# USTC-StarTeam/DR4SR

Measured on AMD Instinct MI355X. Metric: training sequences/sec, SASRec d=64 L=50, higher is better.
Workload: dtype f32; 1 GPU; SASRec on amazon-toys-shaped synthetic rows (BASELINE configs[1]): N=11925, L=50, d=64, 2 layers, 2 heads, FFN 128, dropout 0.50, B=256 rows/GPU/step, toys histogram (10.9% valid) seqlen; global_batch=256, seq_len=50, parallelism=dp1, hip_graph=True, steps_per_graph=30

## Files before the change

dr4sr_amd/csrc/common.h:

```cpp
#pragma once
#include <hip/hip_runtime.h>
#include <stdint.h>
#include "../../include/dr4sr_hip.h"
#include "../../include/dr4sr_hip_hooks.h"
#include <stdlib.h>
#include <string.h>

#include <atomic>
#include <mutex>
int dr4sr_env_generation();
std::mutex& dr4sr_env_mutex();
#define DR4SR_ENV(NAME) ([]() -> const char* {                                                   \
    static std::atomic<int> gen_{-1}; static bool set_ = false; static char buf_[256];           \
    const int cur_ = dr4sr_env_generation();                                                     \
    if (gen_.load(std::memory_order_acquire) != cur_) {                                          \
        std::lock_guard<std::mutex> lk_(dr4sr_env_mutex());                                      \
        if (gen_.load(std::memory_order_relaxed) != cur_) { const char* e_ = getenv(NAME); set_ = e_ != nullptr; \
            if (e_) { strncpy(buf_, e_, sizeof(buf_) - 1); buf_[sizeof(buf_) - 1] = 0; }         \
            gen_.store(cur_, std::memory_order_release); } }                                     \
    return set_ ? buf_ : nullptr; }())

#ifdef DR4SR_EXPERIMENTS
#define DR4SR_XENV(NAME) DR4SR_ENV(NAME)
#else
// ... 506 lines not shown
        const int lane = threadIdx.x & 63, w = threadIdx.x >> 6, r16 = lane & 15, g = lane >> 4;
#pragma unroll
        for (int i = 0; i < N / 64; ++i) {
            const int col = (w + 4 * i) * 16 + r16;
            const float bv = bias ? bias[col] : 0.f;
#pragma unroll
            for (int r = 0; r < BM / 16; ++r)
#pragma unroll
                for (int q = 0; q < 4; ++q) Cs[(r * 16 + 4 * g + q) * ldc + col] = t.a[r][i][q] + bv;
        }
    }
}
template <int BM, int N>
__device__ __forceinline__ void tile_to_global(const TileAcc<BM, N>& t, float* __restrict__ C, int ldc, const float* __restrict__ bias,
                                               int t0, int T) {
    if constexpr (BM == 64) acc_to_global(t.a, C, ldc, bias, t0, T);
    else {
        const int lane = threadIdx.x & 63, w = threadIdx.x >> 6, r16 = lane & 15, g = lane >> 4;
#pragma unroll
        for (int i = 0; i < N / 64; ++i) {
            const int col = (w + 4 * i) * 16 + r16;
            const float bv = bias ? bias[col] : 0.f;
#pragma unroll
            for (int r = 0; r < BM / 16; ++r)
#pragma unroll
                for (int q = 0; q < 4; ++q) {
                    const int tt = t0 + r * 16 + 4 * g + q;
                    if (tt < T) C[(size_t)tt * ldc + col] = t.a[r][i][q] + bv;
                }
        }
    }
}

template <int BM, int K>
__device__ __forceinline__ void load_tile_bm(float* __restrict__ As, int lda, const float* __restrict__ G, int ldg, int t0, int T) {
    constexpr int C4 = K / 4;
    for (int i = threadIdx.x; i < BM * C4; i += 256) {
        const int row = i / C4, c = (i % C4) * 4;
        float4 v = make_float4(0.f, 0.f, 0.f, 0.f);
        if (t0 + row < T) v = ld4(G + (size_t)(t0 + row) * ldg + c);
        st4(As + row * lda + c, v);
    }
}

template <int K>
__device__ __forceinline__ void load_tile(float* __restrict__ As, int lda, const float* __restrict__ G,
                                          int ldg, int t0, int T) {
    constexpr int C4 = K / 4;
    for (int i = threadIdx.x; i < 64 * C4; i += 256) {
        const int row = i / C4, c = (i % C4) * 4;
        float4 v = make_float4(0.f, 0.f, 0.f, 0.f);
        if (t0 + row < T) v = ld4(G + (size_t)(t0 + row) * ldg + c);
        st4(As + row * lda + c, v);
    }
}

template <int NV, bool DPP = false>
__device__ __forceinline__ void ln_stats16(const float4 (&v)[NV], float& mean, float& rstd, float eps) {
    constexpr float invD = 1.0f / (64 * NV);
    float s = 0.f;
#pragma unroll
    for (int j = 0; j < NV; ++j) s += (v[j].x + v[j].y) + (v[j].z + v[j].w);
    mean = group16_sum_sel<DPP>(s) * invD;
    float q = 0.f;
#pragma unroll
    for (int j = 0; j < NV; ++j) {
// ... 66 lines not shown
```

dr4sr_amd/csrc/linear.hip:

```cpp
#include "common.h"
#include "kernels.h"
#include <cstdlib>
#define STAMP(i) do { if (A.stamps && blockIdx.x == 0 && threadIdx.x == 0) A.stamps[i] = __builtin_amdgcn_s_memtime(); } while (0)

extern __shared__ __attribute__((aligned(16))) float smem[];

__global__ __launch_bounds__(256) void k_transpose(const float* __restrict__ params, float* __restrict__ wT,
                                                   int64_t o_in, int64_t o_out, int64_t o_w1, int64_t o_w2,
                                                   int64_t layer_stride, int64_t wT_stride, int D, int F) {
    const int m = blockIdx.y, layer = blockIdx.z;
    const float* src;
    float* dst = wT + layer * wT_stride;
    int R, C;
    if (m == 0) { src = params + o_in + layer * layer_stride; R = 3 * D; C = D; }
    else if (m == 1) { src = params + o_out + layer * layer_stride; R = D; C = D; dst += 3 * D * D; }
    else if (m == 2) { src = params + o_w1 + layer * layer_stride; R = F; C = D; dst += 4 * D * D; }
    else { src = params + o_w2 + layer * layer_stride; R = D; C = F; dst += 4 * D * D + D * F; }
    for (int i = blockIdx.x * 256 + threadIdx.x; i < R * C; i += gridDim.x * 256) {
        const int r = i / C, c = i % C;
        dst[c * R + r] = src[i];
    }
}

int launch_transpose_weights(const dr4sr_sasrec_plan* p, const Workspace& ws, hipStream_t s) {
// ... 166 lines not shown
        const int layer = j / E4, q = j % E4, e = 4 * q;
        int64_t so; int C, m_off;
        if (e < 3 * D * D) { so = o_in; C = D; m_off = 0; }
        else if (e < 4 * D * D) { so = o_out; C = D; m_off = 3 * D * D; }
        else if (e < 4 * D * D + F * D) { so = o_w1; C = D; m_off = 4 * D * D; }
        else { so = o_w2; C = F; m_off = 4 * D * D + F * D; }
        const int K = C, idx = q - m_off / 4, lane = idx & 63, tq = idx >> 6, ci = tq % (K / 16), ct = tq / (K / 16);
        const int n = ct * 16 + (lane & 15), k0 = (lane >> 4) * (K / 4) + 4 * ci;
        st4(out + (size_t)layer * E + e, ld4(A.E + so + layer * LSTR + (size_t)n * C + k0));
    }
}
template <int D>
__global__ __launch_bounds__(256) void k_wfrag_write(const EmbQkvArgs A) { wfrag_image_write<D>(A); }
int launch_wfrag_write(const dr4sr_sasrec_plan* p, const Workspace& ws, hipStream_t s) {
    EmbQkvArgs A{};
    A.E = p->params + ws.off[0]; A.W = p->params + poff(ws, 0, P_IN_W); A.wf_layers = p->n_layer;
    A.sp = reinterpret_cast<const unsigned short*>(ws.wfrag);
    hipLaunchKernelGGL(k_wfrag_write<128>, dim3(64), dim3(256), 0, s, A);
    return DR4SR_LAUNCH_CHECK();
}

template <int BM, int D>
__global__ __launch_bounds__(256) void k_embqkv_fwd(const EmbQkvArgs A) {
    constexpr int N = 3 * D, LDA = D + 4, LPT = D / 4, TPB = 256 / LPT;
    if constexpr (BM == 16 && D == 128) { if (A.wf_layers > 0) wfrag_image_write<D>(A); }
    const int T = A.state[DR4SR_STATE_T], t0 = xcd_tile(T, BM, A.xcd) * BM;
    if (t0 >= T) return;
    float* As = smem;
    const int c = (threadIdx.x % LPT) * 4;
    const bool dodrop = A.training && A.p > 0.f;
    const RngKey rk = make_rng(A.seed, (uint32_t)A.state[DR4SR_STATE_RNGSTEP], A.p);
    constexpr bool PFE = BM == 16 && D == 64;
    WFragT<PFE ? D : 16, PFE ? N : 64> f_in;
    if constexpr (PFE) wfrag_load(f_in, A.W, D);
    const int bh = A.tile_seq[t0 >> 4];
#pragma unroll
    for (int r0 = 0; r0 < BM; r0 += TPB) {
        const int r = r0 + threadIdx.x / LPT, t = t0 + r;
        if (r < BM) {
            float4 o = make_float4(0.f, 0.f, 0.f, 0.f);
            if (t < T) {
                const int b = find_seq_from(A.cu, A.B, t, bh), pos = t - A.cu[b];
                const int64_t row = A.rows ? A.rows[b] : b;
                int64_t id = A.idx[row * A.L + pos];
                if (A.idx32 && c == 0) A.idx32[t] = (id > 0 && id < A.n_items) ? (int)id : 0;
                if (A.tok && c == 0) A.tok[t] = make_int2(t - pos, b | ((A.cu[b + 1] - A.cu[b]) << 20) | (id == 0 ? 1 << 30 : 0));
                id = id < 0 ? 0 : (id >= A.n_items ? A.n_items - 1 : id);
                o = ld4(A.E + id * D + c);
                const float4 pe = ld4(A.P + (size_t)pos * D + c);
                o = make_float4(o.x + pe.x, o.y + pe.y, o.z + pe.z, o.w + pe.w);
                if (dodrop) {
                    const float4 m = drop4(rk, DR4SR_SITE_EMB, ((uint64_t)b * A.L + pos) * D + c);
                    o.x *= m.x; o.y *= m.y; o.z *= m.z; o.w *= m.w;
                }
                st4(A.X + (size_t)t * D + c, o);
            }
            st4(As + r * LDA + c, o);
        }
    }
    lds_barrier();
    TileAcc<BM, N> acc;
    tile_zero(acc);
    if constexpr (PFE) tile_mma_frag<BM, D, N>(As, LDA, f_in, acc);
    else tile_gemm<D == 128 && BM == 32, BM, D, N>(As, LDA, A.W, D, false, A.sp, WSplitGeo<D, 128>::E, 0, acc);
    tile_to_global<BM, N>(acc, A.QKV, N, A.bias, t0, T);
    if (A.dqkv_zero) zero_kv_rows<BM, D>(A.dqkv_zero, t0, T);
}

int launch_embqkv_fwd(const dr4sr_sasrec_plan* p, const Workspace& ws, int training, hipStream_t s) {
    const int D = p->D, bm = tile_rows(ws);
    const size_t lds = sizeof(float) * bm * (D + 4);
    dim3 grid((ws.Tmax + bm - 1) / bm), blk(256);
    EmbQkvArgs A;
    A.E = p->params + ws.off[0]; A.P = p->params + ws.off[1]; A.idx = p->in_item_id; A.rows = p->rows; A.cu = ws.cu; A.tile_seq = ws.tile_seq; A.X = ws.X[0];
    A.W = p->params + poff(ws, 0, P_IN_W); A.bias = p->params + poff(ws, 0, P_IN_B); A.QKV = ws.layer[0].qkv; A.state = p->state;
    A.B = p->B; A.L = p->L; A.n_items = p->n_items; A.training = training; A.seed = p->seed; A.p = p->p_drop;
    A.idx32 = de_owner_mode(ws) ? ws.idx32 : nullptr;
    A.sp = wsplit_of(p, ws, 0); A.wf_layers = 0;
    if (wfrag_img_on(p, ws)) { A.sp = reinterpret_cast<const unsigned short*>(ws.wfrag); A.wf_layers = p->n_layer; }
    const bool in_tile = attn_in_tile(p, ws);
    A.tok = (in_tile || ws.attn_tile_sa || attn_wave_on(p, ws)) ? ws.tok : nullptr; A.dqkv_zero = in_tile ? ws.layer[0].dqkv : nullptr;
    A.xcd = tile_xcd_order(p, ws) ? 1 : 0;
    if (A.xcd) grid.x = xcd_grid((int)grid.x, bm);
    if (wave_tiles(p, ws)) return launch_wt_embqkv_fwd(A, ws.Tmax, s);
#define EQ(B_) do { if (D == 64) hipLaunchKernelGGL((k_embqkv_fwd<B_, 64>), grid, blk, lds, s, A); \
                    else hipLaunchKernelGGL((k_embqkv_fwd<B_, 128>), grid, blk, lds, s, A); } while (0)
    BM_DISPATCH(bm, EQ);
#undef EQ
    return DR4SR_LAUNCH_CHECK();
}


struct LnCarry { float4 v; float mean, rstd; uint32_t keep; };
template <int F>
struct RowCarry { LnCarry ln1, ln2; float4 a[F / 64]; uint32_t akeep; };
__host__ __device__ constexpr bool carry_vals(int CARRY) { return CARRY != 0; }
__host__ __device__ constexpr bool carry_bits(int CARRY) { return CARRY == 1 || CARRY == 3; }
__device__ __forceinline__ uint32_t keep_bits4(const float4& m) {
    return (m.x != 0.f ? 1u : 0u) | (m.y != 0.f ? 2u : 0u) | (m.z != 0.f ? 4u : 0u) | (m.w != 0.f ? 8u : 0u);
}
__device__ __forceinline__ float4 keep_factors4(const RngKey& k, uint32_t bits) {
    return make_float4((bits & 1u) ? k.scale : 0.f, (bits & 2u) ? k.scale : 0.f, (bits & 4u) ? k.scale : 0.f, (bits & 8u) ? k.scale : 0.f);
}

template <int BM, int D, bool RES_IN_LDS, bool COPY_LDS, bool CARRY = false, bool KPRE = false, bool NOST = false>
__device__ __forceinline__ void ln_rowpass(const float* __restrict__ Cs, int ldc, const float* res, int ldres,
                                           const float* __restrict__ lnw, const float* __restrict__ lnb, float eps,
                                           float* __restrict__ U, float* __restrict__ OUT, float* __restrict__ ST,
                                           float* Ls, int ldl, int t0, int T, bool dodrop, const RngKey& rk,
                                           uint32_t site, float4 (*yreg)[D / 64] = nullptr, LnCarry* cy = nullptr) {
    constexpr int NV = D / 64, PASSES = BM / 16;
    static_assert(!CARRY || (NV == 1 && PASSES == 1), "the carried row state is one float4 per thread");
    static_assert(!KPRE || CARRY, "the keep bits arrive in the carried row state");
    static_assert(!NOST || CARRY, "the row state leaves through *cy only");
    const int l16 = threadIdx.x & 15, rsub = threadIdx.x >> 4;
    float4 gam[NV], bet[NV], v[PASSES][NV];
    float mean[PASSES], rstd[PASSES];
#pragma unroll
    for (int j = 0; j < NV; ++j) { gam[j] = ld4(lnw + 4 * l16 + 64 * j); bet[j] = ld4(lnb + 4 * l16 + 64 * j); }
#pragma unroll
    for (int ps = 0; ps < PASSES; ++ps) {
        const int row = ps * 16 + rsub, t = t0 + row;
        const bool ok = t < T;
#pragma unroll
        for (int j = 0; j < NV; ++j) {
            const int c = 4 * l16 + 64 * j;
            float4 o = ld4(Cs + row * ldc + c);
            float4 r = make_float4(0.f, 0.f, 0.f, 0.f);
            if (RES_IN_LDS) r = ld4(res + row * ldres + c);
            else if constexpr (KPRE) r = cy->v;
            else if (ok) r = ld4(res + (size_t)t * ldres + c);
            if (dodrop) {
                float4 m;
                if constexpr (KPRE) m = keep_factors4(rk, cy->keep); else m = drop4(rk, site, (uint64_t)t * D + c);
                o.x *= m.x; o.y *= m.y; o.z *= m.z; o.w *= m.w;
                if constexpr (CARRY && !KPRE) cy->keep = keep_bits4(m);
            }
            v[ps][j] = make_float4(r.x + o.x, r.y + o.y, r.z + o.z, r.w + o.w);
            if constexpr (!NOST) { if (ok) st4(U + (size_t)t * D + c, v[ps][j]); }
        }
    }
#pragma unroll
    for (int ps = 0; ps < PASSES; ++ps) ln_stats16<NV, NV == 1>(v[ps], mean[ps], rstd[ps], eps);
    if constexpr (CARRY) { cy->v = v[0][0]; cy->mean = mean[0]; cy->rstd = rstd[0]; }
#pragma unroll
    for (int ps = 0; ps < PASSES; ++ps) {
        const int row = ps * 16 + rsub, t = t0 + row;
        const bool ok = t < T;
#pragma unroll
        for (int j = 0; j < NV; ++j) {
            const int c = 4 * l16 + 64 * j;
            const float m = mean[ps], rs = rstd[ps];
            const float4 yv = make_float4((v[ps][j].x - m) * rs * gam[j].x + bet[j].x, (v[ps][j].y - m) * rs * gam[j].y + bet[j].y,
                                          (v[ps][j].z - m) * rs * gam[j].z + bet[j].z, (v[ps][j].w - m) * rs * gam[j].w + bet[j].w);
            if (ok && OUT) st4(OUT + (size_t)t * D + c, yv);
            if (yreg) yreg[ps][j] = ok ? yv : make_float4(0.f, 0.f, 0.f, 0.f);
            if (COPY_LDS) st4(Ls + row * ldl + c, ok ? yv : make_float4(0.f, 0.f, 0.f, 0.f));
        }
        if constexpr (!NOST) { if (ok && l16 == 0) { ST[2 * (size_t)t] = mean[ps]; ST[2 * (size_t)t + 1] = rstd[ps]; } }
    }
}

template <int F>
__device__ __forceinline__ void row_keep_store(const PostArgs& A, const RowCarry<F>& cy, const int t0, const int T) {
    static_assert(F == 128, "16 bits per thread");
    const int t = t0 + (threadIdx.x >> 4);
    if (t < T) A.row_keep[16 * (size_t)t + (threadIdx.x & 15)] = (unsigned short)(cy.ln1.keep | (cy.ln2.keep << 4) | (cy.akeep << 8));
}
__device__ __forceinline__ uint32_t row_keep_word(const RngKey& rk, const uint32_t sP, const uint32_t sF, const uint32_t sA, const bool actdrop, const int t) {
    constexpr int D = 64, F = 128;
    const int l16 = threadIdx.x & 15, pr = l16 >> 1;
    const bool odd = l16 & 1;
    const uint32_t b0 = drop_bits8(rk, odd ? sF : sP, (uint64_t)t * D + 8 * pr);
    const uint32_t b1 = actdrop ? drop_bits8(rk, sA, (uint64_t)t * F + (odd ? 64 : 0) + 8 * pr) : 0xffu;
    const uint32_t own0 = odd ? b0 >> 4 : b0 & 15u, own1 = odd ? b1 >> 4 : b1 & 15u;
    const uint32_t give = odd ? (b0 & 15u) | ((b1 & 15u) << 4) : (b0 >> 4) | (b1 & 0xf0u);
    const uint32_t got = lane_xor1_u32(give), got0 = got & 15u, got1 = got >> 4;
    return odd ? got0 | (own0 << 4) | (got1 << 8) | (own1 << 12) : own0 | (got0 << 4) | (own1 << 8) | (got1 << 12);
}
template <int BM, int D, int F, bool FFN_ONLY, bool KEEPQ = false, int CARRY = 0, bool KU = false>
__device__ __forceinline__ void post_fwd_body(const PostArgs& A, const int t0, const int T, float4 (*zreg)[D / 64] = nullptr,
                                              tattn::Keep* keep_out = nullptr, RowCarry<F>* cy = nullptr) {
    constexpr int LD = D + 4, LF = F + 4, NVF = F / 64, PASSES = BM / 16;
    float* R0 = smem;
    float* R1 = R0 + BM * LD;
    float* R2 = R1 + BM * LD;
    const int l16 = threadIdx.x & 15, rsub = threadIdx.x >> 4;
    const bool dodrop = A.training && A.p > 0.f;
    const RngKey rk = make_rng(A.seed, (uint32_t)A.state[DR4SR_STATE_RNGSTEP], A.p);
    const uint32_t sP = A.sP, sA = A.sA, sF = A.sF;
    const bool actdrop = dodrop && sA != 0xffffffffu;

    constexpr bool PF = BM == 16 && !FFN_ONLY;
    WFragT<PF ? D : 16, PF ? D : 64> f_out;
    WFragT<PF ? D : 16, PF ? F : 64> f_w1;
    WFragT<PF ? F : 16, PF ? D : 64> f_w2;
    WFragT<PF ? D : 16, PF ? 3 * D : 64> f_nx;
    STAMP(0);
    static_assert(!KU || (BM == 16 && D == 64 && F == 128 && !FFN_ONLY && CARRY != 0), "one row, one float4, 16 keep bits per thread");
    constexpr bool NOST = CARRY == 1;
    auto keep_upfront = [&]() {
        if constexpr (KU) {
            const uint32_t w = row_keep_word(rk, sP, sF, sA, actdrop, t0 + rsub);
            cy->ln1.keep = w & 15u; cy->ln2.keep = (w >> 4) & 15u; cy->akeep = w >> 8;
        }
    };
    if constexpr (KU) {
        const int t = t0 + rsub;
        cy->ln1.v = t < T ? ld4(A.x + (size_t)t * D + 4 * l16) : make_float4(0.f, 0.f, 0.f, 0.f);
        __builtin_amdgcn_sched_barrier(0);
    }
    if (FFN_ONLY) {
        load_tile_bm<BM, D>(R1, LD, A.x, D, t0, T);
    } else {
        constexpr bool AT = BM == 16 && (D == 64 || D == 128);
        bool at_on = false;
        if constexpr (AT) at_on = A.at.on != 0;
        if (!at_on) load_tile_bm<BM, D>(R0, LD, A.ctx, D, t0, T);
        tattn::FwdPre<AT ? D : 64, KEEPQ> att_pre;
#ifdef DR4SR_WFRAG_UPFRONT
        constexpr bool SPREAD = false;
#else
        constexpr bool SPREAD = AT && PF;
#endif
        constexpr bool KU_EARLY = KU && SPREAD;
        if constexpr (SPREAD) {
            if (at_on) {
                tattn::fwd_issue<D, KEEPQ>(A, t0, T, att_pre);
                __builtin_amdgcn_sched_barrier(0);
                { if constexpr (D == 128) wfrag_load_img(f_out, reinterpret_cast<const float*>(A.sp) + WSplitGeo<D, F>::OUT); else wfrag_load(f_out, A.out_w, D); }
                __builtin_amdgcn_sched_barrier(0);
// ... 10 lines not shown
                if (A.nx_qkv) { if constexpr (D == 128) wfrag_load_img(f_nx, reinterpret_cast<const float*>(A.sp) + WSplitGeo<D, F>::E); else wfrag_load(f_nx, A.nx_in_w, D); }
            } else {
                { if constexpr (D == 128) wfrag_load_img(f_out, reinterpret_cast<const float*>(A.sp) + WSplitGeo<D, F>::OUT); else wfrag_load(f_out, A.out_w, D); }
                { if constexpr (D == 128) wfrag_load_img(f_w1, reinterpret_cast<const float*>(A.sp) + WSplitGeo<D, F>::W1); else wfrag_load(f_w1, A.w1, D); }
                { if constexpr (D == 128) wfrag_load_img(f_w2, reinterpret_cast<const float*>(A.sp) + WSplitGeo<D, F>::W2); else wfrag_load(f_w2, A.w2, F); }
                if (A.nx_qkv) { if constexpr (D == 128) wfrag_load_img(f_nx, reinterpret_cast<const float*>(A.sp) + WSplitGeo<D, F>::E); else wfrag_load(f_nx, A.nx_in_w, D); }
                if constexpr (KU_EARLY) keep_upfront();
            }
        } else {
            constexpr bool EARLY = D == 128;
            if constexpr (AT && EARLY) { if (at_on) { tattn::fwd_issue<D, KEEPQ>(A, t0, T, att_pre); __builtin_amdgcn_sched_barrier(0); } }
            if constexpr (PF) {
                { if constexpr (D == 128) wfrag_load_img(f_out, reinterpret_cast<const float*>(A.sp) + WSplitGeo<D, F>::OUT); else wfrag_load(f_out, A.out_w, D); }
                { if constexpr (D == 128) wfrag_load_img(f_w1, reinterpret_cast<const float*>(A.sp) + WSplitGeo<D, F>::W1); else wfrag_load(f_w1, A.w1, D); }
                { if constexpr (D == 128) wfrag_load_img(f_w2, reinterpret_cast<const float*>(A.sp) + WSplitGeo<D, F>::W2); else wfrag_load(f_w2, A.w2, F); }
                if (A.nx_qkv) { if constexpr (D == 128) wfrag_load_img(f_nx, reinterpret_cast<const float*>(A.sp) + WSplitGeo<D, F>::E); else wfrag_load(f_nx, A.nx_in_w, D); }
            }
            if constexpr (AT) {
                if (at_on) {
                    if constexpr (!EARLY) tattn::fwd_issue<D, KEEPQ>(A, t0, T, att_pre);
                    tattn::fwd_stage<D, KEEPQ>(A, t0, T, smem + att_lds_off(D, F), att_pre);
                    const tattn::Keep k = tattn::fwd_compute<D, KEEPQ>(A, t0, T, R0, LD, smem + att_lds_off(D, F), att_pre);
                    if (keep_out) *keep_out = k;
                    if constexpr (CARRY == 2) tattn::keep_store(A.at, k, t0, T);
                }
            }
        }
        lds_barrier(); STAMP(1);
        {
            TileAcc<BM, D> acc;
            tile_zero(acc);
            if constexpr (PF) tile_mma_frag<BM, D, D>(R0, LD, f_out, acc);
            else tile_gemm<BM == 32 && (D == 128 || FFN_ONLY), BM, D, D>(R0, LD, A.out_w, D, false, A.sp, WSplitGeo<D, F>::E, WSplitGeo<D, F>::OUT, acc);
            tile_to_lds<BM, D>(acc, R2, LD, A.out_b);
        }
        lds_barrier(); STAMP(2);
        if constexpr (KU && !KU_EARLY) keep_upfront();
        ln_rowpass<BM, D, false, true, CARRY != 0, KU, NOST>(R2, LD, A.x, D, A.ln1_w, A.ln1_b, A.eps, A.u1, A.y, A.st1, R1, LD, t0, T, dodrop, rk, sP, nullptr,
                                                  CARRY ? &cy->ln1 : nullptr);
    }
    lds_barrier(); STAMP(3);
    {
        TileAcc<BM, F> acc;
        tile_zero(acc);
        if constexpr (PF) tile_mma_frag<BM, D, F>(R1, LD, f_w1, acc);
        else tile_gemm<BM == 32 && (D == 128 || FFN_ONLY), BM, D, F>(R1, LD, A.w1, D, false, A.sp, WSplitGeo<D, F>::E, WSplitGeo<D, F>::W1, acc);
        tile_to_lds<BM, F>(acc, R2, LF, A.b1);
    }
    lds_barrier(); STAMP(4);
    {
        float4 av[PASSES][NVF];
#pragma unroll
        for (int ps = 0; ps < PASSES; ++ps)
#pragma unroll
            for (int j = 0; j < NVF; ++j) av[ps][j] = ld4(R2 + (ps * 16 + rsub) * LF + 4 * l16 + 64 * j);
#pragma unroll
        for (int ps = 0; ps < PASSES; ++ps) {
            const int row = ps * 16 + rsub, t = t0 + row;
            const bool ok = t < T;
#pragma unroll
            for (int j = 0; j < NVF; ++j) {
                const int c = 4 * l16 + 64 * j;
                const float4 a4 = av[ps][j];
                float4 h = make_float4(gelu_erf(a4.x), gelu_erf(a4.y), gelu_erf(a4.z), gelu_erf(a4.w));
                if constexpr (CARRY != 0) { cy->a[j] = a4; if (j == 0 && !KU) cy->akeep = 0; }
                if (actdrop) {
                    float4 m;
                    if constexpr (KU) m = keep_factors4(rk, cy->akeep >> (4 * j)); else m = drop4(rk, sA, (uint64_t)t * F + c);
                    h.x *= m.x; h.y *= m.y; h.z *= m.z; h.w *= m.w;
                    if constexpr (CARRY != 0 && !KU) cy->akeep |= keep_bits4(m) << (4 * j);
                }
                if (ok) { if constexpr (!NOST) st4(A.a + (size_t)t * F + c, a4); st4(A.h + (size_t)t * F + c, h); }
                st4(R2 + row * LF + c, h);
            }
        }
    }
    lds_barrier(); STAMP(5);
    {
        TileAcc<BM, D> acc;
        tile_zero(acc);
        if constexpr (PF) tile_mma_frag<BM, F, D>(R2, LF, f_w2, acc);
        else tile_gemm<BM == 32 && (D == 128 || FFN_ONLY), BM, F, D>(R2, LF, A.w2, F, false, A.sp, WSplitGeo<D, F>::E, WSplitGeo<D, F>::W2, acc);
        tile_to_lds<BM, D>(acc, R0, LD, A.b2);
    }
    lds_barrier(); STAMP(6);
    if (!FFN_ONLY && A.nx_qkv) {
        ln_rowpass<BM, D, true, true, CARRY != 0, KU, NOST>(R0, LD, R1, LD, A.ln2_w, A.ln2_b, A.eps, A.u2, A.z, A.st2, R1, LD, t0, T, dodrop, rk, sF, nullptr,
                                                  CARRY ? &cy->ln2 : nullptr);
        if constexpr (CARRY == 2) row_keep_store<F>(A, *cy, t0, T);
        lds_barrier();
        TileAcc<BM, 3 * D> acc;
        tile_zero(acc);
        if constexpr (PF) tile_mma_frag<BM, D, 3 * D>(R1, LD, f_nx, acc);
        else tile_gemm<BM == 32 && (D == 128 || FFN_ONLY), BM, D, 3 * D>(R1, LD, A.nx_in_w, D, false, A.sp ? A.sp + 4 * WSplitGeo<D, F>::E : nullptr, WSplitGeo<D, F>::E, 0, acc);
        tile_to_global<BM, 3 * D>(acc, A.nx_qkv, 3 * D, A.nx_in_b, t0, T);
        if (A.nx_dqkv_zero) zero_kv_rows<BM, D>(A.nx_dqkv_zero, t0, T);
    } else {
        ln_rowpass<BM, D, true, false, CARRY != 0, KU, NOST>(R0, LD, R1, LD, A.ln2_w, A.ln2_b, A.eps, A.u2, A.z, A.st2, nullptr, 0, t0, T, dodrop, rk, sF, zreg,
                                                   CARRY ? &cy->ln2 : nullptr);
        if constexpr (CARRY == 2) row_keep_store<F>(A, *cy, t0, T);
    }
    STAMP(15);
}

template <int BM, int D, int F, bool FFN_ONLY, bool KB = false>
__global__ __launch_bounds__(256) void k_post_fwd(const PostArgs A) {
    const int T = A.state[DR4SR_STATE_T], t0 = xcd_tile(T, BM, A.xcd) * BM;
    if (t0 >= T) return;
    if constexpr (KB) {
        RowCarry<F> cy;
        cy.ln1.keep = cy.ln2.keep = cy.akeep = 0;
        post_fwd_body<BM, D, F, FFN_ONLY, false, 2, true>(A, t0, T, nullptr, nullptr, &cy);
    } else post_fwd_body<BM, D, F, FFN_ONLY>(A, t0, T);
}

template <int NV, bool DPP = false>
__device__ __forceinline__ void flush_affine(const float4 (&dgam)[NV], const float4 (&dbet)[NV], float* scr, float* dst) {
    constexpr int D = 64 * NV;
    const int l16 = threadIdx.x & 15, lane = threadIdx.x & 63, w = threadIdx.x >> 6;
    auto fold = [&](float v) { if constexpr (DPP) return xrow_sum(v); else return xrow_sum_ref(v); };
#pragma unroll
    for (int j = 0; j < NV; ++j) {
        const int c = 4 * l16 + 64 * j;
        const float4 a = make_float4(fold(dgam[j].x), fold(dgam[j].y), fold(dgam[j].z), fold(dgam[j].w));
        const float4 b = make_float4(fold(dbet[j].x), fold(dbet[j].y), fold(dbet[j].z), fold(dbet[j].w));
        if (lane < 16) { st4(scr + w * 2 * D + c, a); st4(scr + w * 2 * D + D + c, b); }
    }
    lds_barrier();
    for (int i = threadIdx.x; i < 2 * D; i += 256)
        dst[i] = (scr[i] + scr[2 * D + i]) + (scr[4 * D + i] + scr[6 * D + i]);
    lds_barrier();
// ... 36 lines not shown
            else {
                const float4 p0 = ld4(La + row * ldl + c);
                float4 p1 = z4;
                if (SRC == 1) p1 = ld4(Lb + row * ldl + c);
                else if (ok) p1 = ld4(Gg + (size_t)t * D + c);
                g[ps][j] = ok ? make_float4(p0.x + p1.x, p0.y + p1.y, p0.z + p1.z, p0.w + p1.w) : z4;
            }
        }
    }
#pragma unroll
    for (int ps = 0; ps < PASSES; ++ps) ln_bwd_row<NV, NV == 1>(g[ps], u[ps], mean[ps], rstd[ps], gam, dgam, dbet);
#pragma unroll
    for (int ps = 0; ps < PASSES; ++ps) {
        const int row = ps * 16 + rsub, t = t0 + row;
        const bool ok = t < T;
#pragma unroll
        for (int j = 0; j < NV; ++j) {
            const int c = 4 * l16 + 64 * j;
            const float4 du = g[ps][j];
            if (DUg && ok) st4(DUg + (size_t)t * D + c, du);
            if (DUl) st4(DUl + row * ldl + c, du);
            float4 dm = du;
            if (dodrop) {
                float4 m;
                if constexpr (BITS) m = keep_factors4(rk, cy->keep); else m = drop4(rk, site, (uint64_t)t * D + c);
                dm.x *= m.x; dm.y *= m.y; dm.z *= m.z; dm.w *= m.w;
            }
            if (ok) st4(DMg + (size_t)t * D + c, dm);
            st4(DMl + row * ldl + c, dm);
        }
    }
}

template <int BM, int D, int F, bool FFN_ONLY, bool DET = false, int CARRY = 0>
__device__ __forceinline__ void post_bwd_body(const PostArgs& A, const int t0, const int T, const int tile,
                                              const float4 (*dzreg)[D / 64] = nullptr, const tattn::Keep* att_staged = nullptr,
                                              const RowCarry<F>* cy_in = nullptr) {
    constexpr int LD = D + 4, LF = F + 4, NV = D / 64, NVF = F / 64, PASSES = BM / 16;
    float* R1 = smem;
    float* R0 = R1 + BM * LD;
    float* R2 = R0 + BM * LD;
    const int l16 = threadIdx.x & 15, rsub = threadIdx.x >> 4;
    const bool dodrop = A.training && A.p > 0.f;
    const RngKey rk = make_rng(A.seed, (uint32_t)A.state[DR4SR_STATE_RNGSTEP], A.p);
    const uint32_t sP = A.sP, sA = A.sA, sF = A.sF;
    const bool actdrop = dodrop && sA != 0xffffffffu;
    float4 dgam[NV], dbet[NV];
#ifdef DR4SR_BWD_NO_PREFETCH
    constexpr bool PFB = false;
#else
    constexpr bool PFB = BM == 16 && !FFN_ONLY && (D == 64 || D == 128);
#endif
    constexpr bool PF64 = PFB && D == 64, PF128 = PFB && D == 128;
    WFragC<PF64 ? 3 * D : 16, PF64 ? D : 64> fr_up;
    WFragC<PFB ? D : 16, PFB ? F : 64> fr_w2;
    WFragC<PFB ? F : 16, PFB ? D : 64> fr_w1;
    WFragC<PFB ? D : 16, PFB ? D : 64> fr_out;
    constexpr bool AT = BM == 16 && !FFN_ONLY && (D == 64 || D == 128);
    bool at_on = false, at_stage = false;
    tattn::Keep keep{0xffffffffu, 0xffffffffu};
    tattn::Stage<AT ? D : 64, true, true> att_st;
    constexpr int UPQ = AT ? (16 * 3 * D / 4) / 256 : 1;
    float4 updq[UPQ];
    bool up_pre = false;
    RowCarry<F> cy_ld;
    const RowCarry<F>* cy = CARRY >= 2 ? &cy_ld : cy_in;
    if constexpr (AT) {
        at_on = A.at.on != 0;
        at_stage = at_on && !att_staged;
        if (att_staged) keep = *att_staged;
// ... 131 lines not shown
                st4(A.du1 + (size_t)(t0 + row) * D + c, make_float4(p0.x + p1.x, p0.y + p1.y, p0.z + p1.z, p0.w + p1.w));
            }
        }
        return;
    }
    ln_bwd_rowpass<BM, D, 1, CARRY>(nullptr, R0, R1, LD, A.u1, A.st1, A.ln1_w, A.du1, nullptr, A.dout, R1, dgam, dbet, t0, T, dodrop, rk, sP, nullptr,
                                    CARRY ? &cy->ln1 : nullptr);
    flush_affine<NV, NV == 1 && BM == 16 && !FFN_ONLY>(dgam, dbet, R2, A.ln_part + (size_t)tile * 4 * D + 2 * D);
    {
        TileAcc<BM, D> acc;
        tile_zero(acc);
        if constexpr (PFB) tile_mma_frag<BM, D, D>(R1, LD, fr_out, acc);
        else tile_gemm<BM == 32 && (D == 128 || FFN_ONLY), BM, D, D>(R1, LD, A.out_w, D, true, A.sp, WSplitGeo<D, F>::E, WSplitGeo<D, F>::OUT, acc);
        tile_to_lds<BM, D>(acc, R0, LD, nullptr);
    }
    lds_barrier();
    constexpr int C4 = D / 4;
    for (int i = threadIdx.x; i < BM * C4; i += 256) {
        const int row = i / C4, c = (i % C4) * 4;
        const bool ok = t0 + row < T;
        const float4 v = ld4(R0 + row * LD + c);
        if (ok && !at_on) st4(A.dctx + (size_t)(t0 + row) * D + c, v);
        if (A.rd) {
            const int lph = C4 / A.n_head;
            float4 o = make_float4(0.f, 0.f, 0.f, 0.f);
            if (ok) o = ld4(A.ctx + (size_t)(t0 + row) * D + c);
            float d = (v.x * o.x + v.y * o.y) + (v.z * o.z + v.w * o.w);
            if (D == 64 && lph == 8) d = group8_sum(d);
            else for (int off = lph >> 1; off > 0; off >>= 1) d += __shfl_xor(d, off, 64);
            if (ok && (i % C4) % lph == 0) A.rd[(size_t)(t0 + row) * A.n_head + (i % C4) / lph] = d;
            if constexpr (AT) { if (at_on && (i % C4) % lph == 0) tattn::Lds<D>(smem + att_lds_off(D, F)).rd[row * 2 + (i % C4) / lph] = d; }
        }
    }
    if constexpr (AT) {
        if (at_on) {
            STAMP(17);
            lds_barrier();
            if (at_stage) tattn::far_rows_if_needed<D>(A.at, tattn::Lds<D>(smem + att_lds_off(D, F)), t0, T);
            STAMP(18);
            tattn::bwd<D, DET>(A, t0, T, R0, LD, smem + att_lds_off(D, F), keep);
        }
    }
    STAMP(26);
}

template <int BM, int D, int F, bool FFN_ONLY, bool DET = false, bool KB = false>
__global__ __launch_bounds__(256) void k_post_bwd(const PostArgs A) {
    const int T = A.state[DR4SR_STATE_T], bx = xcd_tile(T, BM, A.xcd), t0 = bx * BM;
    if (t0 >= T) return;
    constexpr int CARRY = (BM == 16 && D == 64 && !FFN_ONLY) ? (KB ? 3 : 2) : 0;
    post_bwd_body<BM, D, F, FFN_ONLY, DET, CARRY>(A, t0, T, bx);
}


__device__ __forceinline__ float meta_weight_token(const ScoreTileArgs& S, const float4& q, float lt, int b, int pos, int64_t row, int t,
                                                   int sub, uint32_t step, float4& dzw) {
    constexpr int MD = 64;
    const float* W1 = S.phi;
    const float* b1 = S.phi + MD * MD;
    const float* W2 = b1 + MD;
    const float* b2 = W2 + 2 * MD;
    float pre[4];
#pragma unroll
    for (int k = 0; k < 4; ++k) pre[k] = b1[4 * sub + k];
#pragma unroll
    for (int s = 0; s < 16; ++s) {
// ... 190 lines not shown
};
template <int BM>
__device__ __forceinline__ void score_prefetch(const PostArgs& A, const ScoreTileArgs& S, const int t0, const int T, ScorePre<BM>& P) {
    constexpr int D = 64;
    const int c = (threadIdx.x & 15) * 4, sub = threadIdx.x & 15;
    const RngKey rk = make_rng(A.seed, (uint32_t)A.state[DR4SR_STATE_RNGSTEP], 0.f);
    const int bh = S.tile_seq[t0 >> 4];
#pragma unroll
    for (int ps = 0; ps < ScorePre<BM>::PASSES; ++ps) {
        const int t = t0 + ps * 16 + (threadIdx.x >> 4);
        P.ok[ps] = t < T;
        P.b[ps] = 0; P.pos[ps] = 0; P.n[ps] = 0; P.row[ps] = 0; P.tgt[ps] = 0; P.ng[ps] = 0;
        P.idin[ps] = (S.ent && P.ok[ps]) ? S.idx32[t] : 0;
        P.ep[ps] = make_float4(0.f, 0.f, 0.f, 0.f); P.en[ps] = P.ep[ps];
        if (P.ok[ps]) {
            const int b = find_seq_from(S.cu, S.B, t, bh), c0 = S.cu[b];
            P.b[ps] = b; P.pos[ps] = t - c0; P.n[ps] = S.cu[b + 1] - c0;
            P.row[ps] = S.rows ? S.rows[b] : b;
            P.tgt[ps] = S.target[P.row[ps] * S.L + P.pos[ps]];
            int64_t ng;
            if (S.sample_neg) {
                ng = sample_neg_id(rk, (uint64_t)b * S.L + P.pos[ps], S.n_items);
                if (sub == 0) S.neg_item[(size_t)b * S.L + P.pos[ps]] = ng;
            } else {
                ng = S.neg_item[(size_t)b * S.L + P.pos[ps]];
            }
            P.ng[ps] = ng < 0 ? 0 : (ng >= S.n_items ? S.n_items - 1 : ng);
            if (P.tgt[ps] > 0 && P.tgt[ps] < S.n_items) { P.ep[ps] = ld4(S.E + P.tgt[ps] * D + c); P.en[ps] = ld4(S.E + P.ng[ps] * D + c); }
        }
    }
}
template <int BM, bool META>
__device__ __forceinline__ void score_tile_regs(const PostArgs& A, const ScoreTileArgs& S, const int t0, const int T, const int tile,
                                                const ScorePre<BM>& P, const float4 (*zreg)[1], float4 (*dzreg)[1], float* red, float* lds_tile) {
    int4* lrec = reinterpret_cast<int4*>(red + 8);
    constexpr int D = 64, LPT = 16, LD = D + 4, PASSES = ScorePre<BM>::PASSES;
    const int c = (threadIdx.x & 15) * 4, sub = threadIdx.x & 15;
    const RngKey rk = make_rng(A.seed, (uint32_t)A.state[DR4SR_STATE_RNGSTEP], 0.f);
    float lsum = 0.f, cnt = 0.f;
    float lt_[PASSES], dpos_[PASSES], dneg_[PASSES], wt_[PASSES];
    bool on_[PASSES];
    float4 dzw_[PASSES];
    auto terms = [&](const int ps, float& lt, float& dpos, float& dneg) {
        const float4 q = zreg[ps][0], ep = P.ep[ps], en = P.en[ps];
        const float sp = lane_group_sum<LPT>(q.x * ep.x + q.y * ep.y + q.z * ep.z + q.w * ep.w);
        const float sn = lane_group_sum<LPT>(q.x * en.x + q.y * en.y + q.z * en.z + q.w * en.w);
        lt = softplus_f(-sp) + softplus_f(sn);
        dpos = -sigmoid_f(-sp); dneg = sigmoid_f(sn);
    };
    auto pass1 = [&](const int ps) {
        on_[ps] = false; lt_[ps] = 0.f; dpos_[ps] = 0.f; dneg_[ps] = 0.f; wt_[ps] = 1.0f; dzw_[ps] = make_float4(0.f, 0.f, 0.f, 0.f);
        if (P.ok[ps] && P.tgt[ps] > 0 && P.tgt[ps] < S.n_items) { terms(ps, lt_[ps], dpos_[ps], dneg_[ps]); on_[ps] = true; }
    };
    if constexpr (META) {
#pragma unroll
        for (int ps = 0; ps < PASSES; ++ps) pass1(ps);
    }
    if constexpr (META) {
        if (S.phi) {
            constexpr int MD = 64;
            const float* W1 = S.phi;
            const float* b1 = S.phi + MD * MD;
            const float* W2 = b1 + MD;
            const float* b2 = W2 + 2 * MD;
            float* Zs = lds_tile;
            float* Ps = lds_tile + BM * LD;
            const uint32_t step = (uint32_t)A.state[DR4SR_STATE_RNGSTEP];
// ... 66 lines not shown
            {
                TileAcc<BM, MD> acc;
                tile_zero(acc);
                tile_mma_xw<BM, MD, MD>(Zs, LD, W1, MD, acc);
                tile_to_lds<BM, MD>(acc, Ps, LD, nullptr);
            }
            lds_barrier();
#pragma unroll
            for (int ps = 0; ps < PASSES; ++ps)
                if (on_[ps]) dzw_[ps] = ld4(Ps + (ps * 16 + (threadIdx.x >> 4)) * LD + c);
        }
    }
#pragma unroll
    for (int ps = 0; ps < PASSES; ++ps) {
        float4 dz = make_float4(0.f, 0.f, 0.f, 0.f);
        if (P.ok[ps]) {
            const int t = t0 + ps * 16 + (threadIdx.x >> 4), b = P.b[ps], pos = P.pos[ps], n = P.n[ps];
            const int64_t row = P.row[ps], tgt = P.tgt[ps], ng = P.ng[ps];
            int4 rec = make_int4(0, 0, 0, 0);
            bool on;
            if constexpr (META) on = on_[ps]; else on = tgt > 0 && tgt < S.n_items;
            if (on) {
                const float4 q = zreg[ps][0], ep = P.ep[ps], en = P.en[ps];
                float lt, dpos, dneg, wt = 1.0f;
                float4 dzw = make_float4(0.f, 0.f, 0.f, 0.f);
                if constexpr (META) { lt = lt_[ps]; dpos = dpos_[ps]; dneg = dneg_[ps]; wt = wt_[ps]; dzw = dzw_[ps]; }
                else terms(ps, lt, dpos, dneg);
                if (sub == 0) { lsum += wt * lt; cnt += 1.f; }
                dpos *= wt; dneg *= wt;
                dz = make_float4(dpos * ep.x + dneg * en.x + dzw.x, dpos * ep.y + dneg * en.y + dzw.y, dpos * ep.z + dneg * en.z + dzw.z,
                                 dpos * ep.w + dneg * en.w + dzw.w);
                float* gp = S.dE + tgt * D + c;
                float* gn = S.dE + ng * D + c;
                if (!S.rec) {
                    unsafeAtomicAdd(gp, dpos * q.x); unsafeAtomicAdd(gp + 1, dpos * q.y); unsafeAtomicAdd(gp + 2, dpos * q.z); unsafeAtomicAdd(gp + 3, dpos * q.w);
                    unsafeAtomicAdd(gn, dneg * q.x); unsafeAtomicAdd(gn + 1, dneg * q.y); unsafeAtomicAdd(gn + 2, dneg * q.z); unsafeAtomicAdd(gn + 3, dneg * q.w);
                } else if (sub == 0) {
                    rec = make_int4((int)tgt, (int)ng, __float_as_int(dpos), __float_as_int(dneg));
                }
            }
            if (S.rec && sub == 0) { if (S.ent) lrec[ps * 16 + (threadIdx.x >> 4)] = rec; else S.rec[t] = rec; }
            if (S.ent && sub == 1) reinterpret_cast<int*>(lrec + BM)[ps * 16 + (threadIdx.x >> 4)] = P.idin[ps];
            if (pos == n - 1) {
                for (int l = n + sub; l < S.L; l += LPT) {
                    const int64_t tl = S.target[row * S.L + l];
                    if (S.sample_neg) S.neg_item[(size_t)b * S.L + l] = sample_neg_id(rk, (uint64_t)b * S.L + l, S.n_items);
                    if (tl > 0 && tl < S.n_items) { lsum += 2.0f * 0.69314718055994530942f; cnt += 1.f; }
                }
            }
        }
        dzreg[ps][0] = dz;
    }
    cnt = wave_sum_dpp(cnt); lsum = wave_sum_dpp(lsum);
    if ((threadIdx.x & 63) == 0) { red[2 * (threadIdx.x >> 6)] = cnt; red[2 * (threadIdx.x >> 6) + 1] = lsum; }
    lds_barrier();
    if (threadIdx.x == 0) {
        S.part[2 * tile] = (red[0] + red[2]) + (red[4] + red[6]);
        S.part[2 * tile + 1] = (red[1] + red[3]) + (red[5] + red[7]);
    }
}

template <int BM, int D, int F, bool META, bool DET = false, bool KU = false>
__device__ __forceinline__ void post_mid_body(const PostArgs& A, const ScoreTileArgs& S) {
    const int T = A.state[DR4SR_STATE_T], bx = xcd_tile(T, BM, A.xcd), t0 = bx * BM;
    if (t0 >= T) return;
    if constexpr (BM != 16) { if (S.ent) tile_sort_init<BM>(S, smem + post_lds_floats(D, F, BM) + 8); }
    if constexpr (D == 64) {
        ScorePre<BM> P;
        if constexpr (BM == 16) score_prefetch<BM>(A, S, t0, T, P);
        float4 zreg[BM / 16][1], dzreg[BM / 16][1];
        PostArgs Af = A;
        if (!S.rec) Af.z = nullptr;
        tattn::Keep keep{0xffffffffu, 0xffffffffu};
        constexpr int CARRY = BM == 16 ? 1 : 0;
        if constexpr (CARRY == 1) Af.u1 = Af.st1 = Af.a = Af.u2 = Af.st2 = nullptr;
        RowCarry<F> cy;
        post_fwd_body<BM, D, F, false, true, CARRY, KU>(Af, t0, T, zreg, &keep, &cy);
        if constexpr (BM != 16) score_prefetch<BM>(A, S, t0, T, P);
        if constexpr (META) lds_barrier();
        score_tile_regs<BM, META>(A, S, t0, T, bx, P, zreg, dzreg, smem + post_lds_floats(D, F, BM), smem);
        if constexpr (BM != 16) { if (S.ent) tile_sort<BM>(S, bx, t0, T, smem + post_lds_floats(D, F, BM) + 8); }
        post_bwd_body<BM, D, F, false, DET, CARRY>(A, t0, T, bx, dzreg, &keep, &cy);
    } else {
        tattn::Keep keep{0xffffffffu, 0xffffffffu};
        post_fwd_body<BM, D, F, false, true>(A, t0, T, nullptr, &keep);
        __syncthreads();
        score_tile<BM, D, META>(A, S, t0, T, bx, smem + post_lds_floats(D, F, BM) + 8);
        if constexpr (BM != 16) { if (S.ent) tile_sort<BM>(S, bx, t0, T, smem + post_lds_floats(D, F, BM) + 8); }
        __syncthreads();
        post_bwd_body<BM, D, F, false, DET>(A, t0, T, bx, nullptr, &keep);
    }
}
template <int BM, int D, int F, bool META, bool DET = false, bool KU = false>
__global__ __launch_bounds__(256) void k_post_mid(const PostArgs A, const ScoreTileArgs S) { post_mid_body<BM, D, F, META, DET, KU>(A, S); }
template <int D, int F>
__global__ __launch_bounds__(256) __attribute__((amdgpu_waves_per_eu(4, 4))) void k_post_mid32(const PostArgs A, const ScoreTileArgs S) {
    post_mid_body<32, D, F, false>(A, S);
}

PostArgs make_post_args(const dr4sr_sasrec_plan* p, const Workspace& ws, int layer, int training) {
    PostArgs A;
    const LayerWs& lw = ws.layer[layer];
    const float* P = p->params;
    A.ctx = lw.ctx; A.x = ws.X[layer];
    A.out_w = P + poff(ws, layer, P_OUT_W); A.out_b = P + poff(ws, layer, P_OUT_B);
    A.ln1_w = P + poff(ws, layer, P_LN1_W); A.ln1_b = P + poff(ws, layer, P_LN1_B);
    A.w1 = P + poff(ws, layer, P_W1); A.b1 = P + poff(ws, layer, P_B1);
    A.w2 = P + poff(ws, layer, P_W2); A.b2 = P + poff(ws, layer, P_B2);
    A.ln2_w = P + poff(ws, layer, P_LN2_W); A.ln2_b = P + poff(ws, layer, P_LN2_B);
    A.u1 = lw.u1; A.y = lw.y; A.st1 = lw.st1; A.a = lw.a; A.h = lw.h; A.u2 = lw.u2; A.st2 = lw.st2; A.z = ws.X[layer + 1];
    A.dz = ws.dX[layer + 1];
    const float* wT = ws.wT + layer * ws.wT_stride;
    const int D = p->D, F = p->F;
    A.out_wT = wT + 3 * D * D; A.w1T = wT + 4 * D * D; A.w2T = wT + 4 * D * D + D * F;
    A.df = lw.df; A.da = lw.da; A.du1 = lw.du1; A.dout = lw.dout; A.dctx = ws.dctx;
// ... 1097 lines not shown
```

Baseline: 2.838 million sequences/s.

## Preload bias and LN params at kernel entry; defer embedding-grad atomics into backward

For BM=16, D=64 tiles, biases and layernorm gamma/beta are loaded into registers at kernel entry instead of being re-read from global memory at each epilogue, which hides their load latency behind earlier work. The scorer's embedding-gradient atomic adds are also stashed in a struct and issued later, midway through the post-backward body, so they overlap with backward compute instead of stalling the scorer. This raises register pressure and reorders the atomics, which could hurt occupancy or change float summation order.

```diff
diff --git a/dr4sr_amd/csrc/common.h b/dr4sr_amd/csrc/common.h
--- a/dr4sr_amd/csrc/common.h
+++ b/dr4sr_amd/csrc/common.h
@@ -562,6 +562,49 @@
     }
 }
 
+__host__ __device__ constexpr bool entry_params(int BM, int D, bool FFN_ONLY) {
+#ifdef DR4SR_NO_ENTRY_PARAMS
+    return false;
+#else
+    return BM == 16 && D == 64 && !FFN_ONLY;
+#endif
+}
+template <int N>
+__device__ __forceinline__ void bias_cols_load(float (&bv)[N / 64], const float* __restrict__ bias) {
+    const int lane = threadIdx.x & 63, w = threadIdx.x >> 6, r16 = lane & 15;
+#pragma unroll
+    for (int i = 0; i < N / 64; ++i) bv[i] = bias[(w + 4 * i) * 16 + r16];
+}
+template <int BM, int N>
+__device__ __forceinline__ void tile_to_lds(const TileAcc<BM, N>& t, float* __restrict__ Cs, int ldc, const float (&bv)[N / 64]) {
+    static_assert(BM == 16 || BM == 32, "the 16x16x4 accumulator layout");
+    const int lane = threadIdx.x & 63, w = threadIdx.x >> 6, r16 = lane & 15, g = lane >> 4;
+#pragma unroll
+    for (int i = 0; i < N / 64; ++i) {
+        const int col = (w + 4 * i) * 16 + r16;
+#pragma unroll
+        for (int r = 0; r < BM / 16; ++r)
+#pragma unroll
+            for (int q = 0; q < 4; ++q) Cs[(r * 16 + 4 * g + q) * ldc + col] = t.a[r][i][q] + bv[i];
+    }
+}
+template <int BM, int N>
+__device__ __forceinline__ void tile_to_global(const TileAcc<BM, N>& t, float* __restrict__ C, int ldc, const float (&bv)[N / 64], int t0, int T) {
+    static_assert(BM == 16 || BM == 32, "the 16x16x4 accumulator layout");
+    const int lane = threadIdx.x & 63, w = threadIdx.x >> 6, r16 = lane & 15, g = lane >> 4;
+#pragma unroll
+    for (int i = 0; i < N / 64; ++i) {
+        const int col = (w + 4 * i) * 16 + r16;
+#pragma unroll
+        for (int r = 0; r < BM / 16; ++r)
+#pragma unroll
+            for (int q = 0; q < 4; ++q) {
+                const int tt = t0 + r * 16 + 4 * g + q;
+                if (tt < T) C[(size_t)tt * ldc + col] = t.a[r][i][q] + bv[i];
+            }
+    }
+}
+
 template <int BM, int K>
 __device__ __forceinline__ void load_tile_bm(float* __restrict__ As, int lda, const float* __restrict__ G, int ldg, int t0, int T) {
     constexpr int C4 = K / 4;
diff --git a/dr4sr_amd/csrc/linear.hip b/dr4sr_amd/csrc/linear.hip
--- a/dr4sr_amd/csrc/linear.hip
+++ b/dr4sr_amd/csrc/linear.hip
@@ -222,6 +222,9 @@
     const RngKey rk = make_rng(A.seed, (uint32_t)A.state[DR4SR_STATE_RNGSTEP], A.p);
     constexpr bool PFE = BM == 16 && D == 64;
     WFragT<PFE ? D : 16, PFE ? N : 64> f_in;
+    float in_b[N / 64];
+    constexpr bool EPB = PFE && entry_params(BM, D, false);
+    if constexpr (EPB) bias_cols_load<N>(in_b, A.bias);
     if constexpr (PFE) wfrag_load(f_in, A.W, D);
     const int bh = A.tile_seq[t0 >> 4];
 #pragma unroll
@@ -253,7 +256,7 @@
     tile_zero(acc);
     if constexpr (PFE) tile_mma_frag<BM, D, N>(As, LDA, f_in, acc);
     else tile_gemm<D == 128 && BM == 32, BM, D, N>(As, LDA, A.W, D, false, A.sp, WSplitGeo<D, 128>::E, 0, acc);
-    tile_to_global<BM, N>(acc, A.QKV, N, A.bias, t0, T);
+    if constexpr (EPB) tile_to_global<BM, N>(acc, A.QKV, N, in_b, t0, T); else tile_to_global<BM, N>(acc, A.QKV, N, A.bias, t0, T);
     if (A.dqkv_zero) zero_kv_rows<BM, D>(A.dqkv_zero, t0, T);
 }
 
@@ -293,21 +296,26 @@
     return make_float4((bits & 1u) ? k.scale : 0.f, (bits & 2u) ? k.scale : 0.f, (bits & 4u) ? k.scale : 0.f, (bits & 8u) ? k.scale : 0.f);
 }
 
-template <int BM, int D, bool RES_IN_LDS, bool COPY_LDS, bool CARRY = false, bool KPRE = false, bool NOST = false>
+template <int BM, int D, bool RES_IN_LDS, bool COPY_LDS, bool CARRY = false, bool KPRE = false, bool NOST = false, bool GPRE = false>
 __device__ __forceinline__ void ln_rowpass(const float* __restrict__ Cs, int ldc, const float* res, int ldres,
                                            const float* __restrict__ lnw, const float* __restrict__ lnb, float eps,
                                            float* __restrict__ U, float* __restrict__ OUT, float* __restrict__ ST,
                                            float* Ls, int ldl, int t0, int T, bool dodrop, const RngKey& rk,
-                                           uint32_t site, float4 (*yreg)[D / 64] = nullptr, LnCarry* cy = nullptr) {
+                                           uint32_t site, float4 (*yreg)[D / 64] = nullptr, LnCarry* cy = nullptr,
+                                           const float4* gb = nullptr) {
     constexpr int NV = D / 64, PASSES = BM / 16;
     static_assert(!CARRY || (NV == 1 && PASSES == 1), "the carried row state is one float4 per thread");
+    static_assert(!GPRE || NV == 1, "gamma and beta arrive as one float4 each");
     static_assert(!KPRE || CARRY, "the keep bits arrive in the carried row state");
     static_assert(!NOST || CARRY, "the row state leaves through *cy only");
     const int l16 = threadIdx.x & 15, rsub = threadIdx.x >> 4;
     float4 gam[NV], bet[NV], v[PASSES][NV];
     float mean[PASSES], rstd[PASSES];
 #pragma unroll
-    for (int j = 0; j < NV; ++j) { gam[j] = ld4(lnw + 4 * l16 + 64 * j); bet[j] = ld4(lnb + 4 * l16 + 64 * j); }
+    for (int j = 0; j < NV; ++j) {
+        if constexpr (GPRE) { gam[j] = gb[0]; bet[j] = gb[1]; }
+        else { gam[j] = ld4(lnw + 4 * l16 + 64 * j); bet[j] = ld4(lnb + 4 * l16 + 64 * j); }
+    }
 #pragma unroll
     for (int ps = 0; ps < PASSES; ++ps) {
         const int row = ps * 16 + rsub, t = t0 + row;
@@ -368,6 +376,10 @@
     const uint32_t got = lane_xor1_u32(give), got0 = got & 15u, got1 = got >> 4;
     return odd ? got0 | (own0 << 4) | (got1 << 8) | (own1 << 12) : own0 | (got0 << 4) | (own1 << 8) | (got1 << 12);
 }
+template <int D, int F>
+struct EntryParams { float out_b[D / 64], b1[F / 64], b2[D / 64], nx_b[3 * D / 64]; float4 ln1[2], ln2[2]; };
+struct NoEntryParams {};
+
 template <int BM, int D, int F, bool FFN_ONLY, bool KEEPQ = false, int CARRY = 0, bool KU = false>
 __device__ __forceinline__ void post_fwd_body(const PostArgs& A, const int t0, const int T, float4 (*zreg)[D / 64] = nullptr,
                                               tattn::Keep* keep_out = nullptr, RowCarry<F>* cy = nullptr) {
@@ -387,6 +399,15 @@
     WFragT<PF ? F : 16, PF ? D : 64> f_w2;
     WFragT<PF ? D : 16, PF ? 3 * D : 64> f_nx;
     STAMP(0);
+    constexpr bool EP = entry_params(BM, D, FFN_ONLY);
+    std::conditional_t<EP, EntryParams<D, F>, NoEntryParams> ep;
+    if constexpr (EP) {
+        bias_cols_load<D>(ep.out_b, A.out_b); bias_cols_load<F>(ep.b1, A.b1); bias_cols_load<D>(ep.b2, A.b2);
+        if (A.nx_qkv) bias_cols_load<3 * D>(ep.nx_b, A.nx_in_b);
+        ep.ln1[0] = ld4(A.ln1_w + 4 * l16); ep.ln1[1] = ld4(A.ln1_b + 4 * l16);
+        ep.ln2[0] = ld4(A.ln2_w + 4 * l16); ep.ln2[1] = ld4(A.ln2_b + 4 * l16);
+        __builtin_amdgcn_sched_barrier(0);
+    }
     static_assert(!KU || (BM == 16 && D == 64 && F == 128 && !FFN_ONLY && CARRY != 0), "one row, one float4, 16 keep bits per thread");
     constexpr bool NOST = CARRY == 1;
     auto keep_upfront = [&]() {
@@ -463,11 +484,13 @@
             tile_zero(acc);
             if constexpr (PF) tile_mma_frag<BM, D, D>(R0, LD, f_out, acc);
             else tile_gemm<BM == 32 && (D == 128 || FFN_ONLY), BM, D, D>(R0, LD, A.out_w, D, false, A.sp, WSplitGeo<D, F>::E, WSplitGeo<D, F>::OUT, acc);
-            tile_to_lds<BM, D>(acc, R2, LD, A.out_b);
+            if constexpr (EP) tile_to_lds<BM, D>(acc, R2, LD, ep.out_b); else tile_to_lds<BM, D>(acc, R2, LD, A.out_b);
         }
         lds_barrier(); STAMP(2);
         if constexpr (KU && !KU_EARLY) keep_upfront();
-        ln_rowpass<BM, D, false, true, CARRY != 0, KU, NOST>(R2, LD, A.x, D, A.ln1_w, A.ln1_b, A.eps, A.u1, A.y, A.st1, R1, LD, t0, T, dodrop, rk, sP, nullptr,
+        if constexpr (EP) ln_rowpass<BM, D, false, true, CARRY != 0, KU, NOST, EP>(R2, LD, A.x, D, A.ln1_w, A.ln1_b, A.eps, A.u1, A.y, A.st1, R1, LD, t0, T, dodrop, rk, sP, nullptr,
+                                                  CARRY ? &cy->ln1 : nullptr, ep.ln1);
+        else ln_rowpass<BM, D, false, true, CARRY != 0, KU, NOST>(R2, LD, A.x, D, A.ln1_w, A.ln1_b, A.eps, A.u1, A.y, A.st1, R1, LD, t0, T, dodrop, rk, sP, nullptr,
                                                   CARRY ? &cy->ln1 : nullptr);
     }
     lds_barrier(); STAMP(3);
@@ -476,7 +499,7 @@
         tile_zero(acc);
         if constexpr (PF) tile_mma_frag<BM, D, F>(R1, LD, f_w1, acc);
         else tile_gemm<BM == 32 && (D == 128 || FFN_ONLY), BM, D, F>(R1, LD, A.w1, D, false, A.sp, WSplitGeo<D, F>::E, WSplitGeo<D, F>::W1, acc);
-        tile_to_lds<BM, F>(acc, R2, LF, A.b1);
+        if constexpr (EP) tile_to_lds<BM, F>(acc, R2, LF, ep.b1); else tile_to_lds<BM, F>(acc, R2, LF, A.b1);
     }
     lds_barrier(); STAMP(4);
     {
@@ -512,11 +535,13 @@
         tile_zero(acc);
         if constexpr (PF) tile_mma_frag<BM, F, D>(R2, LF, f_w2, acc);
         else tile_gemm<BM == 32 && (D == 128 || FFN_ONLY), BM, F, D>(R2, LF, A.w2, F, false, A.sp, WSplitGeo<D, F>::E, WSplitGeo<D, F>::W2, acc);
-        tile_to_lds<BM, D>(acc, R0, LD, A.b2);
+        if constexpr (EP) tile_to_lds<BM, D>(acc, R0, LD, ep.b2); else tile_to_lds<BM, D>(acc, R0, LD, A.b2);
     }
     lds_barrier(); STAMP(6);
     if (!FFN_ONLY && A.nx_qkv) {
-        ln_rowpass<BM, D, true, true, CARRY != 0, KU, NOST>(R0, LD, R1, LD, A.ln2_w, A.ln2_b, A.eps, A.u2, A.z, A.st2, R1, LD, t0, T, dodrop, rk, sF, nullptr,
+        if constexpr (EP) ln_rowpass<BM, D, true, true, CARRY != 0, KU, NOST, EP>(R0, LD, R1, LD, A.ln2_w, A.ln2_b, A.eps, A.u2, A.z, A.st2, R1, LD, t0, T, dodrop, rk, sF, nullptr,
+                                                  CARRY ? &cy->ln2 : nullptr, ep.ln2);
+        else ln_rowpass<BM, D, true, true, CARRY != 0, KU, NOST>(R0, LD, R1, LD, A.ln2_w, A.ln2_b, A.eps, A.u2, A.z, A.st2, R1, LD, t0, T, dodrop, rk, sF, nullptr,
                                                   CARRY ? &cy->ln2 : nullptr);
         if constexpr (CARRY == 2) row_keep_store<F>(A, *cy, t0, T);
         lds_barrier();
@@ -524,10 +549,12 @@
         tile_zero(acc);
         if constexpr (PF) tile_mma_frag<BM, D, 3 * D>(R1, LD, f_nx, acc);
         else tile_gemm<BM == 32 && (D == 128 || FFN_ONLY), BM, D, 3 * D>(R1, LD, A.nx_in_w, D, false, A.sp ? A.sp + 4 * WSplitGeo<D, F>::E : nullptr, WSplitGeo<D, F>::E, 0, acc);
-        tile_to_global<BM, 3 * D>(acc, A.nx_qkv, 3 * D, A.nx_in_b, t0, T);
+        if constexpr (EP) tile_to_global<BM, 3 * D>(acc, A.nx_qkv, 3 * D, ep.nx_b, t0, T); else tile_to_global<BM, 3 * D>(acc, A.nx_qkv, 3 * D, A.nx_in_b, t0, T);
         if (A.nx_dqkv_zero) zero_kv_rows<BM, D>(A.nx_dqkv_zero, t0, T);
     } else {
-        ln_rowpass<BM, D, true, false, CARRY != 0, KU, NOST>(R0, LD, R1, LD, A.ln2_w, A.ln2_b, A.eps, A.u2, A.z, A.st2, nullptr, 0, t0, T, dodrop, rk, sF, zreg,
+        if constexpr (EP) ln_rowpass<BM, D, true, false, CARRY != 0, KU, NOST, EP>(R0, LD, R1, LD, A.ln2_w, A.ln2_b, A.eps, A.u2, A.z, A.st2, nullptr, 0, t0, T, dodrop, rk, sF, zreg,
+                                                   CARRY ? &cy->ln2 : nullptr, ep.ln2);
+        else ln_rowpass<BM, D, true, false, CARRY != 0, KU, NOST>(R0, LD, R1, LD, A.ln2_w, A.ln2_b, A.eps, A.u2, A.z, A.st2, nullptr, 0, t0, T, dodrop, rk, sF, zreg,
                                                    CARRY ? &cy->ln2 : nullptr);
         if constexpr (CARRY == 2) row_keep_store<F>(A, *cy, t0, T);
     }
@@ -630,10 +657,20 @@
     }
 }
 
+struct TableAdds {
+    float* gp; float* gn; float dpos, dneg; float4 q;
+    __device__ __forceinline__ void issue() const {
+        if (gp) {
+            unsafeAtomicAdd(gp, dpos * q.x); unsafeAtomicAdd(gp + 1, dpos * q.y); unsafeAtomicAdd(gp + 2, dpos * q.z); unsafeAtomicAdd(gp + 3, dpos * q.w);
+            unsafeAtomicAdd(gn, dneg * q.x); unsafeAtomicAdd(gn + 1, dneg * q.y); unsafeAtomicAdd(gn + 2, dneg * q.z); unsafeAtomicAdd(gn + 3, dneg * q.w);
+        }
+    }
+};
+
 template <int BM, int D, int F, bool FFN_ONLY, bool DET = false, int CARRY = 0>
 __device__ __forceinline__ void post_bwd_body(const PostArgs& A, const int t0, const int T, const int tile,
                                               const float4 (*dzreg)[D / 64] = nullptr, const tattn::Keep* att_staged = nullptr,
-                                              const RowCarry<F>* cy_in = nullptr) {
+                                              const RowCarry<F>* cy_in = nullptr, const TableAdds* ta = nullptr) {
     constexpr int LD = D + 4, LF = F + 4, NV = D / 64, NVF = F / 64, PASSES = BM / 16;
     float* R1 = smem;
     float* R0 = R1 + BM * LD;
@@ -831,6 +868,7 @@
             if constexpr (AT) { if (at_on && (i % C4) % lph == 0) tattn::Lds<D>(smem + att_lds_off(D, F)).rd[row * 2 + (i % C4) / lph] = d; }
         }
     }
+    if constexpr (PF64) { if (ta) { __builtin_amdgcn_sched_barrier(0); ta->issue(); __builtin_amdgcn_sched_barrier(0); } }
     if constexpr (AT) {
         if (at_on) {
             STAMP(17);
@@ -1087,7 +1125,8 @@
 }
 template <int BM, bool META>
 __device__ __forceinline__ void score_tile_regs(const PostArgs& A, const ScoreTileArgs& S, const int t0, const int T, const int tile,
-                                                const ScorePre<BM>& P, const float4 (*zreg)[1], float4 (*dzreg)[1], float* red, float* lds_tile) {
+                                                const ScorePre<BM>& P, const float4 (*zreg)[1], float4 (*dzreg)[1], float* red, float* lds_tile,
+                                                TableAdds* ta = nullptr) {
     int4* lrec = reinterpret_cast<int4*>(red + 8);
     constexpr int D = 64, LPT = 16, LD = D + 4, PASSES = ScorePre<BM>::PASSES;
     const int c = (threadIdx.x & 15) * 4, sub = threadIdx.x & 15;
@@ -1220,7 +1259,9 @@
                                  dpos * ep.w + dneg * en.w + dzw.w);
                 float* gp = S.dE + tgt * D + c;
                 float* gn = S.dE + ng * D + c;
-                if (!S.rec) {
+                if (!S.rec && ta) {
+                    ta->gp = gp; ta->gn = gn; ta->dpos = dpos; ta->dneg = dneg; ta->q = q;
+                } else if (!S.rec) {
                     unsafeAtomicAdd(gp, dpos * q.x); unsafeAtomicAdd(gp + 1, dpos * q.y); unsafeAtomicAdd(gp + 2, dpos * q.z); unsafeAtomicAdd(gp + 3, dpos * q.w);
                     unsafeAtomicAdd(gn, dneg * q.x); unsafeAtomicAdd(gn + 1, dneg * q.y); unsafeAtomicAdd(gn + 2, dneg * q.z); unsafeAtomicAdd(gn + 3, dneg * q.w);
                 } else if (sub == 0) {
@@ -1263,12 +1304,18 @@
         constexpr int CARRY = BM == 16 ? 1 : 0;
         if constexpr (CARRY == 1) Af.u1 = Af.st1 = Af.a = Af.u2 = Af.st2 = nullptr;
         RowCarry<F> cy;
+#ifdef DR4SR_ADDS_IN_SCORER
+        constexpr bool DEFER = false;
+#else
+        constexpr bool DEFER = BM == 16;
+#endif
+        TableAdds ta{nullptr, nullptr, 0.f, 0.f, make_float4(0.f, 0.f, 0.f, 0.f)};
         post_fwd_body<BM, D, F, false, true, CARRY, KU>(Af, t0, T, zreg, &keep, &cy);
         if constexpr (BM != 16) score_prefetch<BM>(A, S, t0, T, P);
         if constexpr (META) lds_barrier();
-        score_tile_regs<BM, META>(A, S, t0, T, bx, P, zreg, dzreg, smem + post_lds_floats(D, F, BM), smem);
+        score_tile_regs<BM, META>(A, S, t0, T, bx, P, zreg, dzreg, smem + post_lds_floats(D, F, BM), smem, DEFER ? &ta : nullptr);
         if constexpr (BM != 16) { if (S.ent) tile_sort<BM>(S, bx, t0, T, smem + post_lds_floats(D, F, BM) + 8); }
-        post_bwd_body<BM, D, F, false, DET, CARRY>(A, t0, T, bx, dzreg, &keep, &cy);
+        post_bwd_body<BM, D, F, false, DET, CARRY>(A, t0, T, bx, dzreg, &keep, &cy, DEFER ? &ta : nullptr);
     } else {
         tattn::Keep keep{0xffffffffu, 0xffffffffu};
         post_fwd_body<BM, D, F, false, true>(A, t0, T, nullptr, &keep);
```

After: 2.989 million sequences/s (median of 6 runs). +5.3%, better.
